# thomasneff/AdaNeRF

Measured on NVIDIA H100. Metric: frames_per_sec_800x800, higher is better.
Workload: dtype bf16

## Files before the change

### adanerf_b200/csrc/api.cu

```cuda
#include <cuda_runtime.h>

#include <algorithm>
#include <cmath>
#include <cstdio>
#include <cstdlib>
#include <cstring>
#include <map>
#include <optional>
#include <string>
#include <vector>

#include "../../include/adanerf_b200.h"
#include "export_loader.h"
#include "flip.cuh"
#include "iwssim.cuh"
#include "mlp.cuh"
#include "ptx.cuh"
#include "stages.cuh"

using namespace adn;

namespace {

struct HostTensor {
// ... 76 lines not shown

adn_status fail(adn_ctx* ctx, adn_status s, const std::string& msg) {
  if (ctx) ctx->last_error = msg;
  return s;
}
adn_status cuda_fail(adn_ctx* ctx, cudaError_t e, const char* where) {
  return fail(ctx, ADN_ERR_CUDA, std::string(where) + ": " + cudaGetErrorString(e));
}
bool joins_group(const adn_ctx* ctx) { return ctx && ctx->sample_budget > 0 && ctx->group.fn; }
adn_status group_fail(adn_ctx* ctx, const char* who) {
  return fail(ctx, ADN_ERR_CUDA, std::string(who) + ": the budget group's reducer returned " + std::to_string(ctx->group.status) +
                                     " in select round " + std::to_string(ctx->group.failed_round));
}
#define ADN_CUDA(ctx, call)                                   \
  do {                                                        \
    cudaError_t e__ = (call);                                 \
    if (e__ != cudaSuccess) return cuda_fail(ctx, e__, #call); \
  } while (0)

class CallOrder {
 public:
  CallOrder(adn_ctx* ctx, cudaStream_t st) : ctx_(ctx), st_(st) {}
  CallOrder(const CallOrder&) = delete;
  CallOrder& operator=(const CallOrder&) = delete;
  ~CallOrder() {
    if (armed_) cudaEventRecord(ctx_->order, st_);
  }
  adn_status begin(const char* who) {
    cudaStreamCaptureStatus cs = cudaStreamCaptureStatusNone;
    const cudaError_t e = cudaStreamIsCapturing(st_, &cs);
    if (e != cudaSuccess) cudaGetLastError();
    if (e != cudaSuccess || cs != cudaStreamCaptureStatusNone)
      return fail(ctx_, ADN_ERR_INVALID, std::string(who) + ": the stream is capturing a CUDA graph; calls cannot be captured "
                                                            "(stage 2's launch epoch and tickets are host state)");
    ADN_CUDA(ctx_, cudaStreamWaitEvent(st_, ctx_->order, 0));
    armed_ = true;
    return ADN_OK;
  }

 private:
  adn_ctx* ctx_;
  cudaStream_t st_;
  bool armed_ = false;
};

adn_status ensure(adn_ctx* ctx, Buf& b, size_t bytes) {
  if (bytes <= b.cap) return ADN_OK;
  ADN_CUDA(ctx, b.release());
  const bool pinned = b.kind == Buf::kPinned;
  const size_t want = pinned ? bytes : bytes + bytes / 8 + 256;
  ADN_CUDA(ctx, pinned ? cudaMallocHost(&b.p, want) : cudaMalloc(&b.p, want));
  b.cap = want;
  return ADN_OK;
}

bool pin_in_place(adn_ctx* ctx, const void* p, size_t bytes) {
  const char* lo = static_cast<const char*>(p);
  for (const adn_ctx::Reg& r : ctx->regs)
    if (lo >= static_cast<const char*>(r.p) && lo + bytes <= static_cast<const char*>(r.p) + r.bytes) return true;
  cudaPointerAttributes attr{};
  if (cudaPointerGetAttributes(&attr, p) == cudaSuccess && attr.type == cudaMemoryTypeHost) return true;
  cudaGetLastError();
  return false;
}

inline uint16_t f2bf(float f) {
  uint32_t u;
  std::memcpy(&u, &f, 4);
  if ((u & 0x7FFFFFFFu) > 0x7F800000u) return uint16_t((u >> 16) | 0x40);
  u += 0x7FFFu + ((u >> 16) & 1u);
  return uint16_t(u >> 16);
}
inline float bf2f(uint16_t h) {
  uint32_t u = uint32_t(h) << 16;
  float f;
  std::memcpy(&f, &u, 4);
  return f;
}

struct Seg {
  int col0, valid;
};

void pack_layer(const float* W, int n_out, int k_in, const std::vector<Seg>& segs, int nsplit, std::vector<uint8_t>& blob) {
  const int n_half = (n_out + 127) / 128;
  for (int nh = 0; nh < n_half; ++nh) {
    for (const Seg& sg : segs) {
      const size_t base = blob.size();
      blob.resize(base + size_t(nsplit) * kBlkBytes, 0);
      for (int n = 0; n < 128; ++n) {
        const int row = nh * 128 + n;
        for (int kk = 0; kk < 64; ++kk) {
          float w = 0.0f;
          if (row < n_out && kk < sg.valid && sg.col0 + kk < k_in) w = W[size_t(row) * k_in + sg.col0 + kk];
          const uint16_t hi = f2bf(w);
          const uint32_t off = sw128_offset(uint32_t(n), uint32_t(kk));
          std::memcpy(&blob[base + off], &hi, 2);
          if (nsplit == 2) {
            const uint16_t lo = f2bf(w - bf2f(hi));
            std::memcpy(&blob[base + kBlkBytes + off], &lo, 2);
          }
        }
      }
    }
  }
}

size_t push_floats(std::vector<float>& f, const float* src, size_t n) {
  while (f.size() % 4) f.push_back(0.0f);
  const size_t off = f.size();
  f.insert(f.end(), src, src + n);
  while (f.size() % 4) f.push_back(0.0f);
  return off;
}

const HostTensor* find(const Net& n, const std::string& name) {
  auto it = n.tensors.find(name);
  return it == n.tensors.end() ? nullptr : &it->second;
}

adn_status upload(adn_ctx* ctx, Net& net, const std::vector<uint8_t>& wblob, const std::vector<float>& fblob) {
  if (fblob.size() > size_t(kSideFloats))
    return fail(ctx, ADN_ERR_INVALID, "network has " + std::to_string(fblob.size()) + " fp32 side parameters (biases and heads), more than " +
                                          std::to_string(kSideFloats) + " fit in shared memory");
  std::memset(net.prog.side, 0, sizeof(net.prog.side));
  std::memcpy(net.prog.side, fblob.data(), fblob.size() * 4);
  adn_status s = ensure(ctx, net.wblob, wblob.size());
  if (s != ADN_OK) return s;
  ADN_CUDA(ctx, cudaMemcpy(net.wblob.p, wblob.data(), wblob.size(), cudaMemcpyHostToDevice));
  return ADN_OK;
}

adn_status build_net0(adn_ctx* ctx) {
  Net& net = ctx->net[0];
  auto bad = [&](const std::string& msg) { return fail(ctx, ADN_ERR_INVALID, "sampling net: " + msg); };
  int D = 0;
  while (find(net, "layers." + std::to_string(D) + ".weight")) ++D;
  if (D < 1 || D > kMaxLayers) return bad("need layers.0.weight .. (1-12 layers)");
  const int nsplit = ctx->mlp0_terms == 3 ? 2 : 1;
  const int width = int(find(net, "layers.0.weight")->rows);
  MlpProgram P{};
  P.n_layers = D;
  std::vector<uint8_t> wblob;
  std::vector<float> fblob;
  int prev = -1;
  for (int l = 0; l < D; ++l) {
    const std::string name = "layers." + std::to_string(l);
    const HostTensor* W = find(net, name + ".weight");
    const HostTensor* B = find(net, name + ".bias");
    if (!B || int64_t(B->data.size()) != W->rows) return bad(name + ".bias is missing or not [" + std::to_string(W->rows) + "]");
    const int n_out = int(W->rows), k_in = int(W->cols);
    const bool last = (l == D - 1);
    if (l == 0) {
      if (k_in < 1 || k_in > 128) return bad(name + ".weight has " + std::to_string(k_in) + " input columns; the input width must be 1-128");
      net.n_in = k_in;
    } else if (k_in != prev) {
      return bad(name + ".weight has " + std::to_string(k_in) + " input columns but layers." + std::to_string(l - 1) + " has " +
                 std::to_string(prev) + " outputs: layer widths must chain (BaseNet skips are not supported)");
    }
    if (!last && n_out != width)
      return bad(name + ".weight has " + std::to_string(n_out) + " outputs; every hidden layer must be as wide as layers.0 (" +
                 std::to_string(width) + ")");
    if (!last && n_out != 128 && n_out != 256)
      return bad(name + ".weight has " + std::to_string(n_out) + " outputs; the hidden width must be 128 or 256");
    if (last && n_out != 128 && n_out != 256)
      return bad(name + ".weight has " + std::to_string(n_out) + " outputs; the output width must be 128 or 256");
    prev = n_out;
    MlpLayer& L = P.layers[l];
    std::vector<Seg> segs;
    if (l == 0) {
      segs = {{0, std::min(64, k_in)}, {64, std::max(0, k_in - 64)}};
    } else {
      for (int c = 0; c < k_in; c += 64) segs.push_back({c, 64});
    }
    L.n_kb = uint8_t(segs.size());
    (l == 0 ? L.in_first : L.n_hid) = L.n_kb;
    for (size_t i = 0; i < segs.size(); ++i) {
      L.k_cnt[i] = uint8_t(std::max(i == 0 ? 1 : 0, (segs[i].valid + 15) / 16));
    }
    L.n_half = uint8_t(n_out / 128);
    L.flags = last ? uint8_t(LF_FINAL_RAW) : uint8_t(LF_RELU | LF_OUT_ACT);
    L.w_off = uint32_t(wblob.size());
    pack_layer(W->data.data(), n_out, k_in, segs, nsplit, wblob);
    L.bias_off = uint32_t(push_floats(fblob, B->data.data(), B->data.size()));
    if (last) {
      net.n_out = n_out;
      P.out_cols = n_out;
    }
  }
  P.in = sampling_tiles(net.n_in, nsplit);
  P.in_nblk0 = P.in.n_blk;
  net.prog = P;
  adn_status s = upload(ctx, net, wblob, fblob);
  if (s != ADN_OK) return s;
  net.depth = D;
  net.width = width;
  net.skip = -1;
  net.ready = true;
  return ADN_OK;
}

adn_status build_net1(adn_ctx* ctx) {
  Net& net = ctx->net[1];
  const int kP = 3 + 6 * ctx->sc.n_freq_pos, kV = 3 + 6 * ctx->sc.n_freq_dir;
  const std::string enc = "posEnc " + (ctx->scene.n_freq_pos < 0 && ctx->scene.n_freq_dir < 0
                                           ? std::string("none")
                                           : std::to_string(ctx->sc.n_freq_pos) + "-" + std::to_string(ctx->sc.n_freq_dir));
  auto bad = [&](const std::string& msg) { return fail(ctx, ADN_ERR_INVALID, "shading net: " + msg); };
  auto shape = [](int64_t r, int64_t c) { return "[" + std::to_string(r) + ", " + std::to_string(c) + "]"; };
  const HostTensor* w0 = find(net, "pts_linears.0.weight");
  if (!w0 || w0->cols != kP)
    return bad("pts_linears.0.weight must be [W, " + std::to_string(kP) + "] (" + enc + ")" +
               (w0 ? ", not " + shape(w0->rows, w0->cols) : std::string(", missing")));
  const int W = int(w0->rows);
  if (W != 128 && W != 256) return bad("pts_linears.0.weight has " + std::to_string(W) + " rows; the width W must be 128 or 256");
  int D = 0;
  while (find(net, "pts_linears." + std::to_string(D) + ".weight")) ++D;
  if (D > kMaxLayers - 2) return bad("pts_linears.0 .. " + std::to_string(D - 1) + ": " + std::to_string(D) + " layers, at most 10 are supported");
  const HostTensor *pw[kMaxLayers], *pb[kMaxLayers];
  int skip = -1;
  for (int i = 0; i < D; ++i) {
    const std::string name = "pts_linears." + std::to_string(i);
    pw[i] = find(net, name + ".weight");
    pb[i] = find(net, name + ".bias");
    if (pw[i]->rows != W) return bad(name + ".weight has " + std::to_string(pw[i]->rows) + " rows; every pts layer must be W = " + std::to_string(W) + " wide");
    if (i > 0 && pw[i]->cols == W + kP) {
      if (skip >= 0)
        return bad(name + ".weight reads cat[pts, h] after the skip at layer " + std::to_string(skip) + "; at most one skip is supported");
      skip = i - 1;
    } else if (i > 0 && pw[i]->cols != W) {
      return bad(name + ".weight has " + std::to_string(pw[i]->cols) + " input columns; expect W = " + std::to_string(W) +
                 " or W + " + std::to_string(kP) + " = " + std::to_string(W + kP) + " (a skip, " + enc + ")");
    }
    if (!pb[i] || int64_t(pb[i]->data.size()) != W) return bad(name + ".bias is missing or not [" + std::to_string(W) + "]");
  }
  struct Want {
    const char* name;
    int64_t rows, cols;
  };
  const Want want[4] = {{"feature_linear", W, W}, {"alpha_linear", 1, W}, {"views_linears.0", W / 2, W + kV}, {"rgb_linear", 3, W / 2}};
  const HostTensor *hw[4], *hb[4];
  for (int j = 0; j < 4; ++j) {
    const std::string name(want[j].name);
    hw[j] = find(net, name + ".weight");
    hb[j] = find(net, name + ".bias");
    if (!hw[j] || hw[j]->rows != want[j].rows || hw[j]->cols != want[j].cols)
      return bad(name + ".weight must be " + shape(want[j].rows, want[j].cols) + " for W = " + std::to_string(W) + " (" + enc + ")" +
                 (hw[j] ? ", not " + shape(hw[j]->rows, hw[j]->cols) : std::string(", missing")));
    if (!hb[j] || int64_t(hb[j]->data.size()) != want[j].rows) return bad(name + ".bias is missing or not [" + std::to_string(want[j].rows) + "]");
  }
  const HostTensor *fw = hw[0], *fb = hb[0], *aw = hw[1], *ab = hb[1], *vw = hw[2], *vb = hb[2], *rw = hw[3], *rb = hb[3];
  net.n_in = kP + kV;
  net.n_out = 4;
  const int nh = W / 64;
  MlpProgram P{};
  P.n_layers = D + 2;
  std::vector<uint8_t> wblob;
  std::vector<float> fblob;
  for (int l = 0; l < D + 2; ++l) {
    MlpLayer& L = P.layers[l];
    std::vector<Seg> segs;
    auto read_p = [&] {
      for (int c = 0; c < kP; c += 64) segs.push_back({c, std::min(64, kP - c)});
      L.in_first = uint8_t(shading_p_blocks(kP));
    };
    auto read_hidden = [&](int col0) {
      for (int b = 0; b < nh; ++b) segs.push_back({col0 + 64 * b, 64});
      L.n_hid = uint8_t(nh);
    };
    const HostTensor *Wt, *B;
    L.n_half = uint8_t(W / 128);
    if (l < D) {
      if (l == 0) {
        read_p();
      } else if (l == skip + 1) {
        read_p();
        read_hidden(kP);
      } else {
        read_hidden(0);
      }
      L.flags = LF_RELU | LF_OUT_ACT | (l == D - 1 ? LF_ALPHA_DOT : 0);
      Wt = pw[l];
      B = pb[l];
    } else if (l == D) {
      read_hidden(0);
      L.flags = LF_OUT_ACT;
      Wt = fw;
      B = fb;
    } else {
      read_hidden(0);
      segs.push_back({W, kV});
      L.in_last = 1;
      L.flags = LF_RELU | LF_FINAL_RGB;
      L.n_half = 1;
      Wt = vw;
      B = vb;
    }
    L.n_kb = uint8_t(segs.size());
    for (size_t i = 0; i < segs.size(); ++i) L.k_cnt[i] = uint8_t((segs[i].valid + 15) / 16);
    L.w_off = uint32_t(wblob.size());
    pack_layer(Wt->data.data(), int(Wt->rows), int(Wt->cols), segs, 1, wblob);
    std::vector<float> bias(size_t(L.n_half) * 128, 0.0f);
    std::copy(B->data.begin(), B->data.end(), bias.begin());
    L.bias_off = uint32_t(push_floats(fblob, bias.data(), bias.size()));
  }
  std::vector<float> rgb_w(3 * 128, 0.0f);
  for (int k = 0; k < 3; ++k) std::copy_n(rw->data.data() + size_t(k) * (W / 2), W / 2, rgb_w.data() + k * 128);
  P.alpha_w_off = uint32_t(push_floats(fblob, aw->data.data(), size_t(W)));
  P.alpha_b_off = uint32_t(push_floats(fblob, ab->data.data(), 1));
  P.rgb_w_off = uint32_t(push_floats(fblob, rgb_w.data(), rgb_w.size()));
  P.rgb_b_off = uint32_t(push_floats(fblob, rb->data.data(), 3));
  P.in = shading_tiles(kP, kV);
  P.in_nblk0 = shading_p_blocks(kP);
  P.out_cols = 4;
  net.prog = P;
  adn_status s = upload(ctx, net, wblob, fblob);
  if (s != ADN_OK) return s;
  net.depth = D;
  net.width = W;
  net.skip = skip;
  net.ready = true;
  return ADN_OK;
}

void set_ndc_projection(adn_ctx* ctx, int W, int H, float focal_in) {
  const double focal = focal_in > 0.0f ? double(focal_in) : 0.5 * double(W) / std::tan(0.5 * double(ctx->scene.fov));
  ctx->sc.ndc_cw = float(-1.0 / (double(W) / (2.0 * focal)));
  ctx->sc.ndc_ch = float(-1.0 / (double(H) / (2.0 * focal)));
}

adn_status ensure_dense_lut(adn_ctx* ctx, int K) {
  if (ctx->dense_K == K) return ADN_OK;
  std::vector<float> lut(K);
  const double max_v = double(ctx->scene.depth_range[1]) - double(ctx->scene.depth_range[0]);
  for (int k = 0; k < K; ++k) {
    const float step = 1.0f / float(K);
    const float lin = (k < (K + 1) / 2) ? float(k) * step : 1.0f - float(K - k) * step;
    const float t = lin + float(0.5 / K);
    const float z = ctx->scene.z_near * (1.0f - t) + ctx->scene.z_far * t;
    const float w = float(std::pow(max_v + 1.0, double(z)));
    lut[k] = ctx->scene.use_ndc ? z : (w - 1.0f) + ctx->scene.depth_range[0];
  }
  adn_status s = ensure(ctx, ctx->zlut_dense, sizeof(float) * K);
  if (s != ADN_OK) return s;
  ADN_CUDA(ctx, cudaMemcpy(ctx->zlut_dense.p, lut.data(), sizeof(float) * K, cudaMemcpyHostToDevice));
  ctx->dense_K = K;
  return ADN_OK;
}

PoseDev make_pose(const float* pose, const float* rot) {
  PoseDev p;
  std::memcpy(p.pose, pose, 12);
  std::memcpy(p.rot, rot, 36);
  return p;
}

std::optional<CameraRays> camera_rays(const adn_ctx* ctx, int W, int H, int row0, int rows) {
  if (!ctx || W < 1 || H < 1 || row0 < 0 || rows < 0 || row0 + rows > H) return std::nullopt;
  CameraRays c;
  const double fov = double(ctx->scene.fov);
  const double focal = 0.5 * W / std::tan(0.5 * fov);
  const double x_dist = std::tan(fov / 2) * focal;
  const double y_dist = x_dist * (double(H) / double(W));
  c.x_pp = x_dist / (W / 2.0);
  c.y_pp = y_dist / (H / 2.0);
  c.start_x = -(x_dist - c.x_pp / 2);
  c.start_y = -(y_dist - c.y_pp / 2);
  c.focal = focal;
  c.W = W;
  c.H = H;
  c.row0 = row0;
  return c;
}

int64_t pad128(int64_t n) { return (n + 127) / 128 * 128; }

adn_status run_mlp(adn_ctx* ctx, int id, const uint8_t* tiles, float* out, const long long* rows_dev, long long rows,
                   cudaStream_t st, const EncodeParams* enc = nullptr) {
  Net& n = ctx->net[id];
  const cudaError_t e = launch_mlp(n.prog, n.wblob.as<uint8_t>(), tiles, out, rows_dev, rows, ctx->d_err, ctx->num_sms, st, enc);
  if (e != cudaSuccess) return cuda_fail(ctx, e, id == 0 ? "launch sampling MLP" : "launch shading MLP");
  ctx->stats.kernel_launches++;
  return ADN_OK;
}
// ... 820 lines not shown
```

### adanerf_b200/csrc/mlp.cu

```cuda
#include <cuda_bf16.h>
#include <cuda_runtime.h>

#include "mlp.cuh"
#include "posenc.cuh"
#include "ptx.cuh"
#include "tiles.cuh"

namespace adn {

template <uint8_t V>
struct ConstFlags {
  __device__ constexpr operator uint8_t() const { return V; }
};

constexpr int kInSlots = 2;

template <int NSPLIT>
struct MlpCfg {
  static constexpr int kNB = (NSPLIT == 2) ? 4 : 2;
  static constexpr int kStageBytes = NSPLIT * kBlkBytes;
  __host__ __device__ static constexpr int stages(int n_blk) { return NSPLIT == 2 ? 2 : (n_blk > 2 ? 6 : 8); }
  __host__ __device__ static constexpr size_t in_bytes(int n_blk) {
    return NSPLIT == 2 ? size_t(NSPLIT) * kNB * kBlkBytes : size_t(kInSlots) * n_blk * kBlkBytes;
  }
  __host__ __device__ static constexpr int n_bars(int n_blk) { return 2 * stages(n_blk) + (NSPLIT == 1 ? 2 * kInSlots : 0); }
  __host__ __device__ static constexpr size_t smem_bytes(int n_blk) {
    return in_bytes(n_blk) + size_t(stages(n_blk)) * kStageBytes + size_t(kSideFloats) * 4 + size_t(n_bars(n_blk)) * 8 +
           1024 ;
  }
  static constexpr size_t kMaxSmemBytes = smem_bytes(2) > smem_bytes(3) ? smem_bytes(2) : smem_bytes(3);
};
static_assert(MlpCfg<1>::kMaxSmemBytes <= 232448 && MlpCfg<2>::kMaxSmemBytes <= 232448, "shared memory per block (sm_90)");

__device__ __forceinline__ void encode_row(const EncodeParams& enc, long long i, long long rows, uint8_t* blk, int row,
                                           bool view) {
  const TileFormat act{1, 2, {0, 64, 0}, {64, 64, 0}};
  const int n_p = 3 + 6 * enc.sc.n_freq_pos;
  zero_row(act, blk, uint32_t(row), 0, view ? 1 : shading_p_blocks(n_p));
  if (i < rows) {
    long long ray;
    float zw;
    if (enc.ray_idx) {
      ray = enc.ray_idx[i];
      zw = enc.z[i];
    } else {
      ray = i / enc.K;
      zw = enc.zlut_dense[i - ray * enc.K];
    }
    float pos[3], dir[3];
    sample_inputs(enc.sc, false, enc.ray_o, enc.ray_d, ray, zw, pos, dir);
    auto put = [&](int j, float v) { put_feature(act, blk, j >> 6, uint32_t(row), j & 63, v); };
    if (view) posenc3_rt(dir, enc.sc.n_freq_dir, put);
    else posenc3_rt(pos, enc.sc.n_freq_pos, put);
  }
}

__device__ __forceinline__ void copy_rows(const uint8_t* __restrict__ src, uint32_t dst, int nblk, int wg, int tw) {
  for (int b = 0; b < nblk; ++b) {
    const uint4* s = reinterpret_cast<const uint4*>(src + size_t(b) * kBlkBytes + size_t(wg) * (kBlkBytes / 2));
    const uint32_t d = dst + uint32_t(b) * kBlkBytes + uint32_t(wg) * (kBlkBytes / 2);
    uint4 v[4];
#pragma unroll
    for (int j = 0; j < 4; ++j) v[j] = __ldg(s + tw + 128 * j);
#pragma unroll
    for (int j = 0; j < 4; ++j) st_shared_v4(d + uint32_t(tw + 128 * j) * 16u, v[j].x, v[j].y, v[j].z, v[j].w);
  }
}

template <int NSPLIT, bool ENC>
__global__ void __launch_bounds__(kMlpThreads, 1)
mlp_kernel(const __grid_constant__ MlpProgram prog, const uint8_t* __restrict__ wblob, const uint8_t* __restrict__ in_tiles,
           float* __restrict__ out, const long long* __restrict__ rows_dev, long long rows_host, int* err_flag,
           const __grid_constant__ EncodeParams enc) {
  static_assert(!ENC || NSPLIT == 1, "fused input encoder: shading net (plain bf16) only");
  using Cfg = MlpCfg<NSPLIT>;
  constexpr int NB = Cfg::kNB;
  const int STAGES = Cfg::stages(prog.in.n_blk);
  constexpr int STAGE_BYTES = Cfg::kStageBytes;
  constexpr int kConsumerWarps = 8, kProducerWarp = 8;
  constexpr int kEncThreads = 96;
  constexpr int kConsumerRegs = ENC ? 232 : 240, kProducerRegs = ENC ? 40 : 24;
  static_assert(2 * kConsumerRegs + kProducerRegs <= 3 * 168, "registers the launch allocates");

  extern __shared__ uint8_t smem_raw[];
  uint8_t* smem = smem_raw + ((1024u - (smem_u32(smem_raw) & 1023u)) & 1023u);
  uint8_t* act = smem;
  uint8_t* ring = act + Cfg::in_bytes(prog.in.n_blk);
  float* side = reinterpret_cast<float*>(ring + size_t(STAGES) * STAGE_BYTES);
  uint64_t* w_full = reinterpret_cast<uint64_t*>(side + kSideFloats);
  uint64_t* w_empty = w_full + STAGES;
  uint64_t* in_full = w_empty + STAGES;
  uint64_t* in_empty = in_full + kInSlots;

  const int warp = __shfl_sync(0xffffffffu, int(threadIdx.x >> 5), 0);
  const int lane = threadIdx.x & 31;
  const long long rows = rows_dev ? *rows_dev : rows_host;
  const long long n_tiles = (rows + kTileM - 1) / kTileM;

  for (int i = threadIdx.x; i < kSideFloats; i += blockDim.x) side[i] = prog.side[i];
  if (threadIdx.x == 0) {
    for (int s = 0; s < STAGES; ++s) {
      mbar_init(&w_full[s], 1);
      mbar_init(&w_empty[s], kConsumerWarps);
    }
    if (NSPLIT == 1) {
      for (int s = 0; s < kInSlots; ++s) {
        mbar_init(&in_full[s], ENC ? kEncThreads : 1);
        mbar_init(&in_empty[s], kConsumerWarps);
      }
    }
    mbar_fence_init();
  }
  __syncthreads();

  if (warp >= kProducerWarp) {
    setmaxnreg_dec<kProducerRegs>();
    if (NSPLIT == 1 && warp > kProducerWarp) {
      if (!ENC && !(warp == kProducerWarp + 1 && lane == 0)) return;
      const uint32_t tile_bytes = prog.in.tile_bytes();
      int slot = 0;
      uint32_t phase = 0;
      for (long long t = blockIdx.x; t < n_tiles; t += gridDim.x) {
        mbar_wait(&in_empty[slot], phase ^ 1, err_flag, 3);
        uint8_t* dst = act + size_t(slot) * tile_bytes;
        if constexpr (ENC) {
          for (int task = int(threadIdx.x) - 32 * (kProducerWarp + 1); task < 2 * kTileM; task += kEncThreads) {
            const int row = task & (kTileM - 1);
            const bool view = task >= kTileM;
            encode_row(enc, t * kTileM + row, rows, dst + (view ? prog.in_nblk0 : 0) * kBlkBytes, row, view);
          }
          fence_proxy_async_smem();
          mbar_arrive(&in_full[slot]);
        } else {
          mbar_arrive_expect_tx(&in_full[slot], tile_bytes);
          bulk_g2s(dst, in_tiles + size_t(t) * tile_bytes, tile_bytes, &in_full[slot]);
        }
        if (++slot == kInSlots) {
          slot = 0;
          phase ^= 1;
        }
      }
      return;
    }
    if (warp == kProducerWarp && lane == 0) {
      int stage = 0;
      uint32_t phase = 0;
      for (long long t = blockIdx.x; t < n_tiles; t += gridDim.x) {
        for (int l = 0; l < prog.n_layers; ++l) {
          const MlpLayer& L = prog.layers[l];
          const int n_st = int(L.n_kb) * int(L.n_half);
          for (int i = 0; i < n_st; ++i) {
            mbar_wait(&w_empty[stage], phase ^ 1, err_flag, 1);
            mbar_arrive_expect_tx(&w_full[stage], STAGE_BYTES);
            bulk_g2s(ring + size_t(stage) * STAGE_BYTES, wblob + L.w_off + size_t(i) * STAGE_BYTES, STAGE_BYTES, &w_full[stage]);
            if (++stage == STAGES) {
              stage = 0;
              phase ^= 1;
            }
          }
        }
      }
    }
    return;
  }

  setmaxnreg_inc<kConsumerRegs>();
  const int wg = warp >> 2;
  const int tw = threadIdx.x & 127;
  const int r0 = 64 * wg + 16 * (warp & 3) + (lane >> 2);
  const int cq = 2 * (lane & 3);
  const int bar_id = 1 + wg;
  const uint32_t act_s = smem_u32(act);
  const uint32_t ring_s = smem_u32(ring);
  const uint32_t wg_off = uint32_t(wg) * (kBlkBytes / 2);
  uint32_t in_s = act_s;
  auto blk_addr = [&](int term, int blk) -> uint32_t { return in_s + uint32_t(term * NB + blk) * kBlkBytes; };
  const uint64_t desc_hi = make_desc_sw128(0) & ~uint64_t(0x3FFF);
  auto desc = [&](uint32_t addr) -> uint64_t { return desc_hi | uint64_t((addr & 0x3FFFF) >> 4); };

  uint32_t afrag[4][4][4];
  auto clear_afrag = [&](int kb0, int kb1) {
#pragma unroll
    for (int kb = 0; kb < 4; ++kb)
#pragma unroll
      for (int k = 0; k < 4; ++k)
#pragma unroll
        for (int j = 0; j < 4; ++j)
          if (kb >= kb0 && kb < kb1) afrag[kb][k][j] = 0u;
  };

  int stage = 0;
  uint32_t phase = 0;
  int prev = -1;
  auto k_block = [&](bool first, int nk, auto mma) {
    mbar_wait(&w_full[stage], phase, err_flag, 2);
    wgmma_fence();
    const uint32_t b = ring_s + uint32_t(stage) * STAGE_BYTES;
#pragma unroll
    for (int k = 0; k < 4; ++k) {
      if (k < nk) mma(k, b, (first && k == 0) ? 0u : 1u);
    }
    wgmma_commit();
    wgmma_wait<1>();
    if (prev >= 0 && lane == 0) mbar_arrive(&w_empty[prev]);
    prev = stage;
    if (++stage == STAGES) {
      stage = 0;
      phase ^= 1;
    }
  };

  int in_slot = 0;
  uint32_t in_phase = 0;
  for (long long t = blockIdx.x; t < n_tiles; t += gridDim.x) {
    if constexpr (NSPLIT == 2) {
#pragma unroll
      for (int term = 0; term < NSPLIT; ++term)
        copy_rows(in_tiles + size_t(t) * prog.in.tile_bytes() + prog.in.blk_off(term, 0), blk_addr(term, 0), prog.in_nblk0, wg, tw);
      fence_proxy_async_smem();
      named_bar_sync(bar_id, 128);
    } else {
      mbar_wait(&in_full[in_slot], in_phase, err_flag, 4);
      in_s = act_s + uint32_t(in_slot) * prog.in.tile_bytes();
      clear_afrag(0, 4);
    }
    float alpha[2] = {0.0f, 0.0f};
    for (int l = 0; l < prog.n_layers; ++l) {
      const MlpLayer& L = prog.layers[l];
      float acc[2][64];
#pragma unroll
      for (int nh = 0; nh < 2; ++nh) {
        if (nh >= L.n_half) break;
        if (NSPLIT == 2) {
          for (int kb = 0; kb < L.n_kb; ++kb) {
            const uint32_t a_hi = blk_addr(0, kb) + wg_off;
            const uint32_t a_lo = a_hi + uint32_t(NB) * kBlkBytes;
            k_block(kb == 0, L.k_cnt[kb], [&](int k, uint32_t b_hi, uint32_t accumulate) {
              const uint32_t b_lo = b_hi + uint32_t(kBlkBytes);
              wgmma_m64n128_bf16(acc[nh], desc(a_hi + 32 * k), desc(b_hi + 32 * k), accumulate);
              wgmma_m64n128_bf16(acc[nh], desc(a_lo + 32 * k), desc(b_hi + 32 * k), 1u);
              wgmma_m64n128_bf16(acc[nh], desc(a_hi + 32 * k), desc(b_lo + 32 * k), 1u);
            });
          }
        } else {
          auto from_smem = [&](int blk) {
            const uint32_t a = blk_addr(0, blk) + wg_off;
            return [&, a](int k, uint32_t b, uint32_t accumulate) {
              wgmma_m64n128_bf16(acc[nh], desc(a + 32 * k), desc(b + 32 * k), accumulate);
            };
          };
#pragma unroll
          for (int ib = 0; ib < NB; ++ib) {
            if (ib >= L.in_first) break;
            k_block(ib == 0, L.k_cnt[ib], from_smem(ib));
          }
#pragma unroll
          for (int hb = 0; hb < 4; ++hb) {
            if (hb >= L.n_hid) break;
            k_block(hb == 0 && L.in_first == 0, 4, [&](int k, uint32_t b, uint32_t accumulate) {
              wgmma_m64n128_bf16_rs(acc[nh], afrag[hb][k], desc(b + 32 * k), accumulate);
            });
          }
          if (L.in_last) k_block(L.n_kb == 1, L.k_cnt[L.n_kb - 1], from_smem(prog.in_nblk0));
        }
      }
      wgmma_wait<0>();
      if (lane == 0) mbar_arrive(&w_empty[prev]);
      prev = -1;
      if constexpr (NSPLIT == 2) {
        named_bar_sync(bar_id, 128);
      } else {
        if (l + 1 == prog.n_layers && lane == 0) mbar_arrive(&in_empty[in_slot]);
      }

      auto epilogue = [&](auto flags) {
        float rgb[2][3] = {{0.f, 0.f, 0.f}, {0.f, 0.f, 0.f}};
        if (NSPLIT == 1 && !(flags & LF_OUT_ACT)) clear_afrag(0, 4);
#pragma unroll
        for (int nh = 0; nh < 2; ++nh) {
          if (nh >= L.n_half) {
            if (NSPLIT == 1 && (flags & LF_OUT_ACT)) clear_afrag(2 * nh, 4);
            break;
          }
#pragma unroll
          for (int i = 0; i < 16; ++i) {
            const int col = nh * 128 + 8 * i + cq;
            const float2 b = *reinterpret_cast<const float2*>(side + L.bias_off + col);
#pragma unroll
            for (int rr = 0; rr < 2; ++rr) {
              const int row = r0 + 8 * rr;
              float v0 = acc[nh][4 * i + 2 * rr] + b.x;
              float v1 = acc[nh][4 * i + 2 * rr + 1] + b.y;
              if (flags & LF_FINAL_RAW) {
                const long long grow = t * kTileM + row;
                if (grow < rows) *reinterpret_cast<float2*>(out + grow * prog.out_cols + col) = make_float2(v0, v1);
                continue;
              }
              if (flags & LF_RELU) {
                v0 = fmaxf(v0, 0.0f);
                v1 = fmaxf(v1, 0.0f);
              }
              if (flags & LF_ALPHA_DOT) {
                const float2 w = *reinterpret_cast<const float2*>(side + prog.alpha_w_off + col);
                alpha[rr] = fmaf(v1, w.y, fmaf(v0, w.x, alpha[rr]));
              }
              if (flags & LF_OUT_ACT) {
                const uint32_t hi = bf16x2(v0, v1);
                if (NSPLIT == 1) {
                  afrag[2 * nh + (i >> 3)][(i >> 1) & 3][2 * (i & 1) + rr] = hi;
                } else {
                  const uint32_t off = uint32_t(col >> 6) * kBlkBytes + sw128_offset(uint32_t(row), uint32_t(col & 63));
                  *reinterpret_cast<uint32_t*>(act + off) = hi;
                  *reinterpret_cast<uint32_t*>(act + NB * kBlkBytes + off) = bf16x2_lo(v0, v1, hi);
                }
              }
              if (flags & LF_FINAL_RGB) {
#pragma unroll
                for (int k = 0; k < 3; ++k) {
                  const float2 w = *reinterpret_cast<const float2*>(side + prog.rgb_w_off + k * 128 + col);
                  rgb[rr][k] = fmaf(v1, w.y, fmaf(v0, w.x, rgb[rr][k]));
                }
              }
            }
          }
        }
        if (flags & LF_FINAL_RGB) {
#pragma unroll
          for (int rr = 0; rr < 2; ++rr) {
            float a = alpha[rr], c0 = rgb[rr][0], c1 = rgb[rr][1], c2 = rgb[rr][2];
#pragma unroll
            for (int m = 1; m <= 2; m <<= 1) {
              a += __shfl_xor_sync(0xffffffffu, a, m);
              c0 += __shfl_xor_sync(0xffffffffu, c0, m);
              c1 += __shfl_xor_sync(0xffffffffu, c1, m);
              c2 += __shfl_xor_sync(0xffffffffu, c2, m);
            }
            const long long grow = t * kTileM + r0 + 8 * rr;
            if ((lane & 3) == 0 && grow < rows)
              reinterpret_cast<float4*>(out)[grow] = make_float4(c0 + side[prog.rgb_b_off], c1 + side[prog.rgb_b_off + 1],
                                                                 c2 + side[prog.rgb_b_off + 2], a + side[prog.alpha_b_off]);
          }
        }
      };
      using F = uint8_t;
      constexpr F kEpiFlags = LF_RELU | LF_ALPHA_DOT | LF_OUT_ACT | LF_FINAL_RAW | LF_FINAL_RGB;
      switch (L.flags & kEpiFlags) {
        case LF_RELU | LF_OUT_ACT: epilogue(ConstFlags<LF_RELU | LF_OUT_ACT>{}); break;
        case LF_RELU | LF_OUT_ACT | LF_ALPHA_DOT: epilogue(ConstFlags<LF_RELU | LF_OUT_ACT | LF_ALPHA_DOT>{}); break;
        case LF_OUT_ACT: epilogue(ConstFlags<LF_OUT_ACT>{}); break;
        case LF_RELU | LF_FINAL_RGB: epilogue(ConstFlags<LF_RELU | LF_FINAL_RGB>{}); break;
        case LF_FINAL_RAW: epilogue(ConstFlags<LF_FINAL_RAW>{}); break;
        default: epilogue(F(L.flags)); break;
      }
      if constexpr (NSPLIT == 2) {
        fence_proxy_async_smem();
        named_bar_sync(bar_id, 128);
      }
    }
    if (NSPLIT == 1 && ++in_slot == kInSlots) {
      in_slot = 0;
      in_phase ^= 1;
    }
  }
}

__global__ void pack_rows_kernel(const float* __restrict__ x, long long rows_host, const long long* __restrict__ rows_dev,
                                 int n_feat, const __grid_constant__ TileFormat fmt, uint8_t* __restrict__ tiles) {
  const long long rows = rows_dev ? *rows_dev : rows_host;
  const long long n_tiles = (rows + kTileM - 1) / kTileM;
  const long long total = n_tiles * kTileM * fmt.n_blk * 8;
  for (long long i = blockIdx.x * (long long)blockDim.x + threadIdx.x; i < total; i += (long long)gridDim.x * blockDim.x) {
    const int chunk = int(i & 7);
    const long long rb = i >> 3;
    const int blk = int(rb % fmt.n_blk);
    const long long row = rb / fmt.n_blk;
    const long long t = row >> 7;
    pack_tile_chunk(fmt, tiles + size_t(t) * fmt.tile_bytes(), blk, uint32_t(row & (kTileM - 1)), chunk,
                    [&](int c) { return row < rows ? x[row * n_feat + c] : 0.0f; });
  }
}

cudaError_t set_max_dyn_smem_once(const void* func, int bytes, unsigned long long* done) {
  int dev = 0;
  cudaError_t e = cudaGetDevice(&dev);
  if (e != cudaSuccess) return e;
  if (dev < 64 && ((__atomic_load_n(done, __ATOMIC_ACQUIRE) >> dev) & 1ull)) return cudaSuccess;
  e = cudaFuncSetAttribute(func, cudaFuncAttributeMaxDynamicSharedMemorySize, bytes);
  if (e != cudaSuccess) return e;
  if (dev < 64) __atomic_fetch_or(done, 1ull << dev, __ATOMIC_RELEASE);
  return cudaSuccess;
}

template <int NSPLIT, bool ENC>
static cudaError_t launch_mlp_t(const MlpProgram& prog, const uint8_t* wblob, const uint8_t* in_tiles, float* out,
                                const long long* rows_dev, long long rows_host, int* err_flag, int num_sms, cudaStream_t stream,
                                const EncodeParams& enc) {
  static unsigned long long attr_done = 0;
  if (prog.in.n_blk < 1 || prog.in.n_blk > 3) return cudaErrorInvalidValue;
  const size_t smem = MlpCfg<NSPLIT>::smem_bytes(prog.in.n_blk);
  auto kernel = mlp_kernel<NSPLIT, ENC>;
  cudaError_t e = set_max_dyn_smem_once(reinterpret_cast<const void*>(kernel), int(MlpCfg<NSPLIT>::kMaxSmemBytes), &attr_done);
  if (e != cudaSuccess) return e;
  long long grid = num_sms;
  if (!rows_dev) {
    const long long n_tiles = (rows_host + kTileM - 1) / kTileM;
    if (n_tiles < grid) grid = n_tiles < 1 ? 1 : n_tiles;
  }
  kernel<<<unsigned(grid), kMlpThreads, smem, stream>>>(prog, wblob, in_tiles, out, rows_dev, rows_host, err_flag, enc);
  return cudaGetLastError();
}

cudaError_t launch_mlp(const MlpProgram& prog, const uint8_t* wblob, const uint8_t* in_tiles, float* out,
                       const long long* rows_dev, long long rows_host, int* err_flag, int num_sms, cudaStream_t stream,
                       const EncodeParams* enc) {
  if (enc) {
    if (prog.in.n_terms != 1) return cudaErrorInvalidValue;
    return launch_mlp_t<1, true>(prog, wblob, in_tiles, out, rows_dev, rows_host, err_flag, num_sms, stream, *enc);
  }
  if (prog.in.n_terms == 2) return launch_mlp_t<2, false>(prog, wblob, in_tiles, out, rows_dev, rows_host, err_flag, num_sms, stream, EncodeParams{});
  return launch_mlp_t<1, false>(prog, wblob, in_tiles, out, rows_dev, rows_host, err_flag, num_sms, stream, EncodeParams{});
}

cudaError_t launch_pack_rows(const float* x, long long rows, const long long* rows_dev, int n_feat, const TileFormat& fmt,
                             uint8_t* tiles, int num_sms, cudaStream_t stream) {
  long long work = ((rows + kTileM - 1) / kTileM) * kTileM * fmt.n_blk * 8;
  int grid = int((work + 255) / 256);
  if (grid < 1) grid = 1;
  if (grid > 16 * num_sms) grid = 16 * num_sms;
  pack_rows_kernel<<<grid, 256, 0, stream>>>(x, rows, rows_dev, n_feat, fmt, tiles);
  return cudaGetLastError();
}

}
```

### adanerf_b200/csrc/mlp.cuh

```cuda
#pragma once
#include <cstdint>
#include <cuda_runtime.h>

#include "stages.cuh"
#include "tiles.cuh"

namespace adn {

constexpr int kMaxLayers = 12;
constexpr int kMlpThreads = 384;
constexpr int kSideFloats = 3592;

enum : uint8_t {
  LF_RELU = 1,
  LF_ALPHA_DOT = 2,
  LF_OUT_ACT = 4,
  LF_FINAL_RAW = 8,
  LF_FINAL_RGB = 16
};

struct MlpLayer {
  uint32_t w_off;
  uint32_t bias_off;
  uint8_t n_kb;
  uint8_t in_first, n_hid, in_last;
  uint8_t n_half;
  uint8_t flags;
  uint8_t k_cnt[6];
};

struct MlpProgram {
  int32_t n_layers;
  TileFormat in;
  int32_t in_nblk0;
  uint32_t alpha_w_off, alpha_b_off, rgb_w_off, rgb_b_off;
  int32_t out_cols;
  MlpLayer layers[kMaxLayers];
  float side[kSideFloats];
};

struct EncodeParams {
  const float* ray_o = nullptr;
  const float* ray_d = nullptr;
  const int32_t* ray_idx = nullptr;
  const float* z = nullptr;
  const float* zlut_dense = nullptr;
  int K = 1;
  SceneDev sc{};
};

cudaError_t set_max_dyn_smem_once(const void* func, int bytes, unsigned long long* done);

cudaError_t launch_mlp(const MlpProgram& prog, const uint8_t* wblob, const uint8_t* in_tiles, float* out,
                       const long long* rows_dev, long long rows_host, int* err_flag, int num_sms, cudaStream_t stream,
                       const EncodeParams* enc = nullptr);
cudaError_t launch_pack_rows(const float* x, long long rows, const long long* rows_dev, int n_feat, const TileFormat& fmt,
                             uint8_t* tiles, int num_sms, cudaStream_t stream);

}
```

### adanerf_b200/csrc/ptx.cuh

```cuda
#pragma once
#include <cstdint>
#include <cuda_runtime.h>

namespace adn {

__device__ __forceinline__ uint32_t smem_u32(const void* p) {
  return static_cast<uint32_t>(__cvta_generic_to_shared(p));
}

__device__ __forceinline__ bool elect_one() {
  uint32_t pred;
  asm volatile("{\n\t.reg .pred p;\n\telect.sync _|p, 0xffffffff;\n\tselp.b32 %0, 1, 0, p;\n\t}" : "=r"(pred));
  return pred != 0;
}

__device__ __forceinline__ void st_shared_v4(uint32_t addr, uint32_t x, uint32_t y, uint32_t z, uint32_t w) {
  asm volatile("st.shared.v4.b32 [%0], {%1, %2, %3, %4};" ::"r"(addr), "r"(x), "r"(y), "r"(z), "r"(w) : "memory");
}

__device__ __forceinline__ float4 ld_shared_f4(uint32_t addr) {
  float4 v;
  asm volatile("ld.shared.v4.f32 {%0, %1, %2, %3}, [%4];" : "=f"(v.x), "=f"(v.y), "=f"(v.z), "=f"(v.w) : "r"(addr));
  return v;
}
// ... 49 lines not shown
  mbar_wait_slow(bar, parity, err_flag, site);
}

__device__ __forceinline__ void bulk_g2s(void* smem_dst, const void* gmem_src, uint32_t bytes, uint64_t* bar) {
  asm volatile("cp.async.bulk.shared::cluster.global.mbarrier::complete_tx::bytes [%0], [%1], %2, [%3];" ::"r"(
                   smem_u32(smem_dst)),
               "l"(gmem_src), "r"(bytes), "r"(smem_u32(bar))
               : "memory");
}
__device__ __forceinline__ void bulk_s2g(void* gmem_dst, const void* smem_src, uint32_t bytes) {
  asm volatile("cp.async.bulk.global.shared::cta.bulk_group [%0], [%1], %2;" ::"l"(gmem_dst), "r"(smem_u32(smem_src)), "r"(bytes)
               : "memory");
}
__device__ __forceinline__ void bulk_commit() { asm volatile("cp.async.bulk.commit_group;" ::: "memory"); }
__device__ __forceinline__ void bulk_wait_read_all() { asm volatile("cp.async.bulk.wait_group.read 0;" ::: "memory"); }
__device__ __forceinline__ void bulk_wait_all() { asm volatile("cp.async.bulk.wait_group 0;" ::: "memory"); }

__device__ __forceinline__ void fence_proxy_async_all() { asm volatile("fence.proxy.async;" ::: "memory"); }
__device__ __forceinline__ void fence_proxy_async_smem() {
  asm volatile("fence.proxy.async.shared::cta;" ::: "memory");
}

template <int N>
__device__ __forceinline__ void setmaxnreg_inc() { asm volatile("setmaxnreg.inc.sync.aligned.u32 %0;" ::"n"(N)); }
template <int N>
__device__ __forceinline__ void setmaxnreg_dec() { asm volatile("setmaxnreg.dec.sync.aligned.u32 %0;" ::"n"(N)); }

__device__ __forceinline__ void wgmma_fence() { asm volatile("wgmma.fence.sync.aligned;" ::: "memory"); }
__device__ __forceinline__ void wgmma_commit() { asm volatile("wgmma.commit_group.sync.aligned;" ::: "memory"); }
template <int N>
__device__ __forceinline__ void wgmma_wait() { asm volatile("wgmma.wait_group.sync.aligned %0;" ::"n"(N) : "memory"); }

__device__ __forceinline__ void wgmma_m64n128_bf16(float (&d)[64], uint64_t a_desc, uint64_t b_desc, uint32_t accumulate) {
  asm volatile(
      "{\n\t.reg .pred p;\n\tsetp.ne.b32 p, %66, 0;\n\t"
      "wgmma.mma_async.sync.aligned.m64n128k16.f32.bf16.bf16 "
      "{%0, %1, %2, %3, %4, %5, %6, %7, %8, %9, %10, %11, %12, %13, %14, %15, "
      "%16, %17, %18, %19, %20, %21, %22, %23, %24, %25, %26, %27, %28, %29, %30, %31, "
      "%32, %33, %34, %35, %36, %37, %38, %39, %40, %41, %42, %43, %44, %45, %46, %47, "
      "%48, %49, %50, %51, %52, %53, %54, %55, %56, %57, %58, %59, %60, %61, %62, %63}, "
      "%64, %65, p, 1, 1, 0, 0;\n\t}"
      : "+f"(d[0]), "+f"(d[1]), "+f"(d[2]), "+f"(d[3]), "+f"(d[4]), "+f"(d[5]), "+f"(d[6]), "+f"(d[7]), "+f"(d[8]),
        "+f"(d[9]), "+f"(d[10]), "+f"(d[11]), "+f"(d[12]), "+f"(d[13]), "+f"(d[14]), "+f"(d[15]), "+f"(d[16]),
        "+f"(d[17]), "+f"(d[18]), "+f"(d[19]), "+f"(d[20]), "+f"(d[21]), "+f"(d[22]), "+f"(d[23]), "+f"(d[24]),
        "+f"(d[25]), "+f"(d[26]), "+f"(d[27]), "+f"(d[28]), "+f"(d[29]), "+f"(d[30]), "+f"(d[31]), "+f"(d[32]),
        "+f"(d[33]), "+f"(d[34]), "+f"(d[35]), "+f"(d[36]), "+f"(d[37]), "+f"(d[38]), "+f"(d[39]), "+f"(d[40]),
        "+f"(d[41]), "+f"(d[42]), "+f"(d[43]), "+f"(d[44]), "+f"(d[45]), "+f"(d[46]), "+f"(d[47]), "+f"(d[48]),
        "+f"(d[49]), "+f"(d[50]), "+f"(d[51]), "+f"(d[52]), "+f"(d[53]), "+f"(d[54]), "+f"(d[55]), "+f"(d[56]),
        "+f"(d[57]), "+f"(d[58]), "+f"(d[59]), "+f"(d[60]), "+f"(d[61]), "+f"(d[62]), "+f"(d[63])
      : "l"(a_desc), "l"(b_desc), "r"(accumulate)
      : "memory");
}

__device__ __forceinline__ void wgmma_m64n128_bf16_rs(float (&d)[64], const uint32_t (&a)[4], uint64_t b_desc, uint32_t accumulate) {
  asm volatile(
      "{\n\t.reg .pred p;\n\tsetp.ne.b32 p, %69, 0;\n\t"
      "wgmma.mma_async.sync.aligned.m64n128k16.f32.bf16.bf16 "
      "{%0, %1, %2, %3, %4, %5, %6, %7, %8, %9, %10, %11, %12, %13, %14, %15, "
      "%16, %17, %18, %19, %20, %21, %22, %23, %24, %25, %26, %27, %28, %29, %30, %31, "
      "%32, %33, %34, %35, %36, %37, %38, %39, %40, %41, %42, %43, %44, %45, %46, %47, "
      "%48, %49, %50, %51, %52, %53, %54, %55, %56, %57, %58, %59, %60, %61, %62, %63}, "
      "{%64, %65, %66, %67}, %68, p, 1, 1, 0;\n\t}"
      : "+f"(d[0]), "+f"(d[1]), "+f"(d[2]), "+f"(d[3]), "+f"(d[4]), "+f"(d[5]), "+f"(d[6]), "+f"(d[7]), "+f"(d[8]),
        "+f"(d[9]), "+f"(d[10]), "+f"(d[11]), "+f"(d[12]), "+f"(d[13]), "+f"(d[14]), "+f"(d[15]), "+f"(d[16]),
        "+f"(d[17]), "+f"(d[18]), "+f"(d[19]), "+f"(d[20]), "+f"(d[21]), "+f"(d[22]), "+f"(d[23]), "+f"(d[24]),
        "+f"(d[25]), "+f"(d[26]), "+f"(d[27]), "+f"(d[28]), "+f"(d[29]), "+f"(d[30]), "+f"(d[31]), "+f"(d[32]),
        "+f"(d[33]), "+f"(d[34]), "+f"(d[35]), "+f"(d[36]), "+f"(d[37]), "+f"(d[38]), "+f"(d[39]), "+f"(d[40]),
        "+f"(d[41]), "+f"(d[42]), "+f"(d[43]), "+f"(d[44]), "+f"(d[45]), "+f"(d[46]), "+f"(d[47]), "+f"(d[48]),
        "+f"(d[49]), "+f"(d[50]), "+f"(d[51]), "+f"(d[52]), "+f"(d[53]), "+f"(d[54]), "+f"(d[55]), "+f"(d[56]),
        "+f"(d[57]), "+f"(d[58]), "+f"(d[59]), "+f"(d[60]), "+f"(d[61]), "+f"(d[62]), "+f"(d[63])
      : "r"(a[0]), "r"(a[1]), "r"(a[2]), "r"(a[3]), "l"(b_desc), "r"(accumulate)
      : "memory");
}

__device__ __forceinline__ uint64_t make_desc_sw128(uint32_t smem_addr_bytes) {
  uint64_t d = 0;
  d |= static_cast<uint64_t>((smem_addr_bytes & 0x3FFFF) >> 4);
  d |= static_cast<uint64_t>(1) << 16;
  d |= static_cast<uint64_t>(1024 >> 4) << 32;
  d |= static_cast<uint64_t>(1) << 62;
  return d;
}

__host__ __device__ __forceinline__ uint32_t sw128_offset(uint32_t row, uint32_t col) {
  const uint32_t chunk = (col >> 3) ^ (row & 7);
  return (row >> 3) * 1024u + (row & 7) * 128u + chunk * 16u + (col & 7) * 2u;
}

}
```

Before: 76.68.

## Split NSPLIT=2 weight stages into 32-column SW64 halves and prefetch input tiles via bulk copy

For the split-precision (hi/lo) path, weights are repacked into 32-column SW64-swizzled stages holding both hi and lo halves in one block-size stage. This allows five ring stages instead of two and finer-grained producer/consumer overlap. The per-thread global-to-shared input copy is replaced by async bulk copies tracked by mbarriers, issued early for the next tile once the last layer no longer needs the input buffer. The cost is more stage handshakes per layer and new descriptor/layout paths that must match exactly.

```diff
diff --git a/adanerf_b200/csrc/api.cu b/adanerf_b200/csrc/api.cu
--- a/adanerf_b200/csrc/api.cu
+++ b/adanerf_b200/csrc/api.cu
@@ -182,23 +182,33 @@
   int col0, valid;
 };
 
-void pack_layer(const float* W, int n_out, int k_in, const std::vector<Seg>& segs, int nsplit, std::vector<uint8_t>& blob) {
+void pack_layer(const float* W, int n_out, int k_in, const std::vector<Seg>& segs, int nsplit, const MlpLayer& L,
+                std::vector<uint8_t>& blob) {
   const int n_half = (n_out + 127) / 128;
+  const int cols = nsplit == 2 ? 16 * stage_k_steps(nsplit) : 64;
+  const uint32_t half = kBlkBytes / 2;
   for (int nh = 0; nh < n_half; ++nh) {
-    for (const Seg& sg : segs) {
-      const size_t base = blob.size();
-      blob.resize(base + size_t(nsplit) * kBlkBytes, 0);
-      for (int n = 0; n < 128; ++n) {
-        const int row = nh * 128 + n;
-        for (int kk = 0; kk < 64; ++kk) {
-          float w = 0.0f;
-          if (row < n_out && kk < sg.valid && sg.col0 + kk < k_in) w = W[size_t(row) * k_in + sg.col0 + kk];
-          const uint16_t hi = f2bf(w);
-          const uint32_t off = sw128_offset(uint32_t(n), uint32_t(kk));
-          std::memcpy(&blob[base + off], &hi, 2);
-          if (nsplit == 2) {
-            const uint16_t lo = f2bf(w - bf2f(hi));
-            std::memcpy(&blob[base + kBlkBytes + off], &lo, 2);
+    for (size_t b = 0; b < segs.size(); ++b) {
+      const Seg& sg = segs[b];
+      const int n_st = nsplit == 2 ? (L.k_cnt[b] + stage_k_steps(nsplit) - 1) / stage_k_steps(nsplit) : 1;
+      for (int s = 0; s < n_st; ++s) {
+        const size_t base = blob.size();
+        blob.resize(base + size_t(nsplit) * (nsplit == 2 ? half : kBlkBytes), 0);
+        for (int n = 0; n < 128; ++n) {
+          const int row = nh * 128 + n;
+          for (int kk = 0; kk < cols; ++kk) {
+            const int c = s * cols + kk;
+            float w = 0.0f;
+            if (row < n_out && c < sg.valid && sg.col0 + c < k_in) w = W[size_t(row) * k_in + sg.col0 + c];
+            const uint16_t hi = f2bf(w);
+            if (nsplit == 2) {
+              const uint32_t off = sw64_offset(uint32_t(n), uint32_t(kk));
+              const uint16_t lo = f2bf(w - bf2f(hi));
+              std::memcpy(&blob[base + off], &hi, 2);
+              std::memcpy(&blob[base + half + off], &lo, 2);
+            } else {
+              std::memcpy(&blob[base + sw128_offset(uint32_t(n), uint32_t(kk))], &hi, 2);
+            }
           }
         }
       }
@@ -281,7 +291,7 @@
     L.n_half = uint8_t(n_out / 128);
     L.flags = last ? uint8_t(LF_FINAL_RAW) : uint8_t(LF_RELU | LF_OUT_ACT);
     L.w_off = uint32_t(wblob.size());
-    pack_layer(W->data.data(), n_out, k_in, segs, nsplit, wblob);
+    pack_layer(W->data.data(), n_out, k_in, segs, nsplit, L, wblob);
     L.bias_off = uint32_t(push_floats(fblob, B->data.data(), B->data.size()));
     if (last) {
       net.n_out = n_out;
@@ -399,7 +409,7 @@
     L.n_kb = uint8_t(segs.size());
     for (size_t i = 0; i < segs.size(); ++i) L.k_cnt[i] = uint8_t((segs[i].valid + 15) / 16);
     L.w_off = uint32_t(wblob.size());
-    pack_layer(Wt->data.data(), int(Wt->rows), int(Wt->cols), segs, 1, wblob);
+    pack_layer(Wt->data.data(), int(Wt->rows), int(Wt->cols), segs, 1, L, wblob);
     std::vector<float> bias(size_t(L.n_half) * 128, 0.0f);
     std::copy(B->data.begin(), B->data.end(), bias.begin());
     L.bias_off = uint32_t(push_floats(fblob, bias.data(), bias.size()));
diff --git a/adanerf_b200/csrc/mlp.cu b/adanerf_b200/csrc/mlp.cu
--- a/adanerf_b200/csrc/mlp.cu
+++ b/adanerf_b200/csrc/mlp.cu
@@ -18,12 +18,12 @@
 template <int NSPLIT>
 struct MlpCfg {
   static constexpr int kNB = (NSPLIT == 2) ? 4 : 2;
-  static constexpr int kStageBytes = NSPLIT * kBlkBytes;
-  __host__ __device__ static constexpr int stages(int n_blk) { return NSPLIT == 2 ? 2 : (n_blk > 2 ? 6 : 8); }
+  static constexpr int kStageBytes = kBlkBytes;
+  __host__ __device__ static constexpr int stages(int n_blk) { return NSPLIT == 2 ? 5 : (n_blk > 2 ? 6 : 8); }
   __host__ __device__ static constexpr size_t in_bytes(int n_blk) {
     return NSPLIT == 2 ? size_t(NSPLIT) * kNB * kBlkBytes : size_t(kInSlots) * n_blk * kBlkBytes;
   }
-  __host__ __device__ static constexpr int n_bars(int n_blk) { return 2 * stages(n_blk) + (NSPLIT == 1 ? 2 * kInSlots : 0); }
+  __host__ __device__ static constexpr int n_bars(int n_blk) { return 2 * stages(n_blk) + (NSPLIT == 1 ? 2 * kInSlots : 2); }
   __host__ __device__ static constexpr size_t smem_bytes(int n_blk) {
     return in_bytes(n_blk) + size_t(stages(n_blk)) * kStageBytes + size_t(kSideFloats) * 4 + size_t(n_bars(n_blk)) * 8 +
            1024 ;
@@ -55,18 +55,6 @@
   }
 }
 
-__device__ __forceinline__ void copy_rows(const uint8_t* __restrict__ src, uint32_t dst, int nblk, int wg, int tw) {
-  for (int b = 0; b < nblk; ++b) {
-    const uint4* s = reinterpret_cast<const uint4*>(src + size_t(b) * kBlkBytes + size_t(wg) * (kBlkBytes / 2));
-    const uint32_t d = dst + uint32_t(b) * kBlkBytes + uint32_t(wg) * (kBlkBytes / 2);
-    uint4 v[4];
-#pragma unroll
-    for (int j = 0; j < 4; ++j) v[j] = __ldg(s + tw + 128 * j);
-#pragma unroll
-    for (int j = 0; j < 4; ++j) st_shared_v4(d + uint32_t(tw + 128 * j) * 16u, v[j].x, v[j].y, v[j].z, v[j].w);
-  }
-}
-
 template <int NSPLIT, bool ENC>
 __global__ void __launch_bounds__(kMlpThreads, 1)
 mlp_kernel(const __grid_constant__ MlpProgram prog, const uint8_t* __restrict__ wblob, const uint8_t* __restrict__ in_tiles,
@@ -77,6 +65,7 @@
   constexpr int NB = Cfg::kNB;
   const int STAGES = Cfg::stages(prog.in.n_blk);
   constexpr int STAGE_BYTES = Cfg::kStageBytes;
+  constexpr int STAGE_K = stage_k_steps(NSPLIT);
   constexpr int kConsumerWarps = 8, kProducerWarp = 8;
   constexpr int kEncThreads = 96;
   constexpr int kConsumerRegs = ENC ? 232 : 240, kProducerRegs = ENC ? 40 : 24;
@@ -108,6 +97,8 @@
         mbar_init(&in_full[s], ENC ? kEncThreads : 1);
         mbar_init(&in_empty[s], kConsumerWarps);
       }
+    } else {
+      for (int g = 0; g < 2; ++g) mbar_init(&in_full[g], 1);
     }
     mbar_fence_init();
   }
@@ -148,7 +139,7 @@
       for (long long t = blockIdx.x; t < n_tiles; t += gridDim.x) {
         for (int l = 0; l < prog.n_layers; ++l) {
           const MlpLayer& L = prog.layers[l];
-          const int n_st = int(L.n_kb) * int(L.n_half);
+          const int n_st = layer_stages(L, NSPLIT);
           for (int i = 0; i < n_st; ++i) {
             mbar_wait(&w_empty[stage], phase ^ 1, err_flag, 1);
             mbar_arrive_expect_tx(&w_full[stage], STAGE_BYTES);
@@ -177,6 +168,8 @@
   auto blk_addr = [&](int term, int blk) -> uint32_t { return in_s + uint32_t(term * NB + blk) * kBlkBytes; };
   const uint64_t desc_hi = make_desc_sw128(0) & ~uint64_t(0x3FFF);
   auto desc = [&](uint32_t addr) -> uint64_t { return desc_hi | uint64_t((addr & 0x3FFFF) >> 4); };
+  const uint64_t desc64_hi = make_desc_sw64(0) & ~uint64_t(0x3FFF);
+  auto desc64 = [&](uint32_t addr) -> uint64_t { return desc64_hi | uint64_t((addr & 0x3FFFF) >> 4); };
 
   uint32_t afrag[4][4][4];
   auto clear_afrag = [&](int kb0, int kb1) {
@@ -197,7 +190,7 @@
     wgmma_fence();
     const uint32_t b = ring_s + uint32_t(stage) * STAGE_BYTES;
 #pragma unroll
-    for (int k = 0; k < 4; ++k) {
+    for (int k = 0; k < STAGE_K; ++k) {
       if (k < nk) mma(k, b, (first && k == 0) ? 0u : 1u);
     }
     wgmma_commit();
@@ -210,15 +203,22 @@
     }
   };
 
+  auto fetch_input = [&](long long tt) {
+    if (tw != 0) return;
+    const uint8_t* src = in_tiles + size_t(tt) * prog.in.tile_bytes() + wg_off;
+    mbar_arrive_expect_tx(&in_full[wg], uint32_t(NSPLIT * prog.in_nblk0) * (kBlkBytes / 2));
+    for (int term = 0; term < NSPLIT; ++term)
+      for (int b = 0; b < prog.in_nblk0; ++b)
+        bulk_g2s(act + size_t(term * NB + b) * kBlkBytes + wg_off, src + prog.in.blk_off(term, b), kBlkBytes / 2, &in_full[wg]);
+  };
+  if (NSPLIT == 2 && blockIdx.x < n_tiles) fetch_input(blockIdx.x);
+
   int in_slot = 0;
   uint32_t in_phase = 0;
   for (long long t = blockIdx.x; t < n_tiles; t += gridDim.x) {
     if constexpr (NSPLIT == 2) {
-#pragma unroll
-      for (int term = 0; term < NSPLIT; ++term)
-        copy_rows(in_tiles + size_t(t) * prog.in.tile_bytes() + prog.in.blk_off(term, 0), blk_addr(term, 0), prog.in_nblk0, wg, tw);
-      fence_proxy_async_smem();
-      named_bar_sync(bar_id, 128);
+      mbar_wait(&in_full[wg], in_phase, err_flag, 4);
+      in_phase ^= 1;
     } else {
       mbar_wait(&in_full[in_slot], in_phase, err_flag, 4);
       in_s = act_s + uint32_t(in_slot) * prog.in.tile_bytes();
@@ -233,14 +233,16 @@
         if (nh >= L.n_half) break;
         if (NSPLIT == 2) {
           for (int kb = 0; kb < L.n_kb; ++kb) {
-            const uint32_t a_hi = blk_addr(0, kb) + wg_off;
-            const uint32_t a_lo = a_hi + uint32_t(NB) * kBlkBytes;
-            k_block(kb == 0, L.k_cnt[kb], [&](int k, uint32_t b_hi, uint32_t accumulate) {
-              const uint32_t b_lo = b_hi + uint32_t(kBlkBytes);
-              wgmma_m64n128_bf16(acc[nh], desc(a_hi + 32 * k), desc(b_hi + 32 * k), accumulate);
-              wgmma_m64n128_bf16(acc[nh], desc(a_lo + 32 * k), desc(b_hi + 32 * k), 1u);
-              wgmma_m64n128_bf16(acc[nh], desc(a_hi + 32 * k), desc(b_lo + 32 * k), 1u);
-            });
+            for (int k0 = 0; k0 < L.k_cnt[kb]; k0 += STAGE_K) {
+              const uint32_t a_hi = blk_addr(0, kb) + wg_off + 32 * k0;
+              const uint32_t a_lo = a_hi + uint32_t(NB) * kBlkBytes;
+              k_block(kb == 0 && k0 == 0, L.k_cnt[kb] - k0, [&](int k, uint32_t b_hi, uint32_t accumulate) {
+                const uint32_t b_lo = b_hi + uint32_t(kBlkBytes / 2);
+                wgmma_m64n128_bf16(acc[nh], desc(a_hi + 32 * k), desc64(b_hi + 32 * k), accumulate);
+                wgmma_m64n128_bf16(acc[nh], desc(a_lo + 32 * k), desc64(b_hi + 32 * k), 1u);
+                wgmma_m64n128_bf16(acc[nh], desc(a_hi + 32 * k), desc64(b_lo + 32 * k), 1u);
+              });
+            }
           }
         } else {
           auto from_smem = [&](int blk) {
@@ -267,8 +269,11 @@
       wgmma_wait<0>();
       if (lane == 0) mbar_arrive(&w_empty[prev]);
       prev = -1;
+      const bool fetch_next = l + 1 == prog.n_layers && t + gridDim.x < n_tiles;
+      const bool fetch_early = fetch_next && !(L.flags & LF_OUT_ACT);
       if constexpr (NSPLIT == 2) {
         named_bar_sync(bar_id, 128);
+        if (fetch_early) fetch_input(t + gridDim.x);
       } else {
         if (l + 1 == prog.n_layers && lane == 0) mbar_arrive(&in_empty[in_slot]);
       }
@@ -355,6 +360,7 @@
       if constexpr (NSPLIT == 2) {
         fence_proxy_async_smem();
         named_bar_sync(bar_id, 128);
+        if (fetch_next && !fetch_early) fetch_input(t + gridDim.x);
       }
     }
     if (NSPLIT == 1 && ++in_slot == kInSlots) {
diff --git a/adanerf_b200/csrc/mlp.cuh b/adanerf_b200/csrc/mlp.cuh
--- a/adanerf_b200/csrc/mlp.cuh
+++ b/adanerf_b200/csrc/mlp.cuh
@@ -29,6 +29,15 @@
   uint8_t k_cnt[6];
 };
 
+__host__ __device__ constexpr int stage_k_steps(int nsplit) { return nsplit == 2 ? 2 : 4; }
+
+__host__ __device__ inline int layer_stages(const MlpLayer& L, int nsplit) {
+  if (nsplit == 1) return int(L.n_kb) * int(L.n_half);
+  int s = 0;
+  for (int kb = 0; kb < L.n_kb; ++kb) s += (L.k_cnt[kb] + stage_k_steps(nsplit) - 1) / stage_k_steps(nsplit);
+  return s * int(L.n_half);
+}
+
 struct MlpProgram {
   int32_t n_layers;
   TileFormat in;
diff --git a/adanerf_b200/csrc/ptx.cuh b/adanerf_b200/csrc/ptx.cuh
--- a/adanerf_b200/csrc/ptx.cuh
+++ b/adanerf_b200/csrc/ptx.cuh
@@ -155,9 +155,23 @@
   return d;
 }
 
+__device__ __forceinline__ uint64_t make_desc_sw64(uint32_t smem_addr_bytes) {
+  uint64_t d = 0;
+  d |= static_cast<uint64_t>((smem_addr_bytes & 0x3FFFF) >> 4);
+  d |= static_cast<uint64_t>(1) << 16;
+  d |= static_cast<uint64_t>(512 >> 4) << 32;
+  d |= static_cast<uint64_t>(2) << 62;
+  return d;
+}
+
 __host__ __device__ __forceinline__ uint32_t sw128_offset(uint32_t row, uint32_t col) {
   const uint32_t chunk = (col >> 3) ^ (row & 7);
   return (row >> 3) * 1024u + (row & 7) * 128u + chunk * 16u + (col & 7) * 2u;
 }
 
+__host__ __device__ __forceinline__ uint32_t sw64_offset(uint32_t row, uint32_t col) {
+  const uint32_t chunk = (col >> 3) ^ ((row >> 1) & 3);
+  return (row >> 3) * 512u + (row & 7) * 64u + chunk * 16u + (col & 7) * 2u;
 }
+
+}
```

Result: faster. 79.96 (median of 6 runs) (+4.3%).
